# cavelandiah/BBMap

Measured on AMD Instinct MI355X. Metric: aligned_reads_per_sec, higher is better.
Workload: dtype int32

## Files before the change

bbmap_amd/csrc/pipeline.hip:

```cpp
#include <hip/hip_runtime.h>

#include <climits>

#include "bbmap_amd.h"
#include "complement.h"
#include "host_common.h"
#include "wave_prims.h"

namespace bbpipe {
using namespace wavep;

__global__ void revcomp_kernel(const bbidx_read *reads, long long n, const uint8_t *in, uint8_t *out) {
    const long long r = (long long)blockIdx.x * (blockDim.x >> 6) + (threadIdx.x >> 6);
    if (r >= n) return;
    const bbidx_read rr = reads[r];
    for (int i = threadIdx.x & 63; i < rr.len; i += 64) out[rr.bases_off + i] = (uint8_t)complement_extended(in[rr.bases_off + rr.len - 1 - i]);
}

struct RescueParams {
    const bbresc_job *jobs;
    const uint8_t *reads;
    const long long *chromOff;
    const int *chromLen, *chromMin;
    const uint8_t *refs;
    bbresc_result *results;
    long long njobs;
    int pointsMatch, pointsMatch2, useAffine, baseHitScore;
};

constexpr int RESC_WAVES = 4, RESC_MAXLEN = 608;

__global__ __launch_bounds__(64 * RESC_WAVES) void quick_rescue_kernel(const RescueParams P) {
    __shared__ __attribute__((aligned(16))) uint8_t rdbuf[RESC_WAVES][RESC_MAXLEN];
    const int wave = __builtin_amdgcn_readfirstlane(threadIdx.x >> 6), lane = threadIdx.x & 63;
    const long long jx = (long long)blockIdx.x * RESC_WAVES + wave;
    if (jx >= P.njobs) return;
    const bbresc_job jb = P.jobs[jx];
    bbresc_result res;
    res.found = 0; res.start = 0; res.stop = 0; res.score = 0; res.mismatches = 0; res.perfect = 0; res.semiperfect = 0; res.maxContig = 0;
    const int len = jb.read_len;
    if (len < 10 || len > RESC_MAXLEN - 8 || jb.chrom < 1) { if (lane == 0) { res.found = len > RESC_MAXLEN - 8 ? -2 : 0; P.results[jx] = res; } return; }
    const uint8_t *bases = P.reads + jb.read_off;
    const uint8_t *ref = P.refs + P.chromOff[jb.chrom];
    const int reflen = P.chromLen[jb.chrom], minIndex = P.chromMin[jb.chrom];
    uint8_t *rd = rdbuf[wave];
    for (int i = lane; i < len; i += 64) rd[i] = bases[i];
    wsync();
    const bool right = (jb.flags & 1) != 0;
    int lower, upper;
    if (right) { lower = max(minIndex, jb.loc); upper = min(reflen - len, jb.loc + jb.searchDist); }
    else { lower = max(minIndex, jb.loc - jb.searchDist); upper = min(reflen - len, jb.loc); }
    int minMM = jb.maxAllowedMismatches + 1, maxContig = 0, bestScore = 0, bestStart = -1, bestAbsdif = INT_MAX;
    bool finished = false;
    for (int base = 0; !finished; base += 64) {
        const int start = right ? lower + base + lane : upper - base - lane;
        const bool valid = start >= lower && start <= upper;
        if (!__ballot(valid)) break;
        const int cap = minMM;
        int mm = 0, contig = 0, cur = 0;
        const int len4 = len & ~3;
        int j = 0;
        for (; j < len4; j += 4) {
            const bool on = valid && mm <= cap;
            if (!__ballot(on)) break;
            const unsigned c4 = *(const unsigned *)(rd + j);
            if (on) {
                unsigned r4;
                __builtin_memcpy(&r4, ref + start + j, 4);
                unsigned x = c4 ^ r4;
                const unsigned isN = c4 ^ 0x4e4e4e4eu;
                const unsigned nz = (((x & 0x7f7f7f7fu) + 0x7f7f7f7fu) | x) & 0x80808080u;
                const unsigned nn = ~((((isN & 0x7f7f7f7fu) + 0x7f7f7f7fu) | isN)) & 0x80808080u;
                const unsigned bad = nz | nn;
                if (bad == 0) cur += 4;
                else {
#pragma unroll
                    for (int q = 0; q < 4; q++) {
                        if (bad & (0x80u << (8 * q))) { mm++; contig = max(contig, cur); cur = 0; } else cur++;
                    }
                }
            }
        }
        for (; j < len; j++) {
            const bool on = valid && mm <= cap;
            if (!__ballot(on)) break;
            const int c = rd[j];
            if (on) {
                const int r = ref[start + j];
                if (c != r || c == 'N') { mm++; contig = max(contig, cur); cur = 0; } else cur++;
            }
        }
        for (u64 m = __ballot(valid && mm <= cap); m; m &= m - 1) {
            const int s = __builtin_ctzll(m);
            const int st = rl(start, s), ms = rl(mm, s), ct = rl(contig, s);
            if (right ? st > upper : st < lower) { finished = true; break; }
            if (ms > minMM) continue;
            const int score = (len - ms) + ct;
            const int ad = st > jb.idealStart ? st - jb.idealStart : jb.idealStart - st;
            if (score > bestScore || (score == bestScore && ad < bestAbsdif)) {
                bestStart = st; minMM = ms; maxContig = ct; bestScore = score; bestAbsdif = ad;
                if (ms == 0) { if (right) upper = min(upper, jb.idealStart + ad); else lower = max(lower, jb.idealStart - ad); }
            }
        }
    }
    if (bestStart >= 0) {
        res.found = 1; res.start = bestStart; res.stop = bestStart + len - 1; res.mismatches = minMM; res.maxContig = maxContig;
        res.score = P.useAffine ? P.pointsMatch + P.pointsMatch2 * (len - 1 - minMM) : maxContig + P.baseHitScore * (len - minMM);
        bool perfect = true;
        int refloc = res.start, readloc = 0, N = 0;
        const int mx = min(res.stop, reflen - 1), nlimit = len / 2;
        if (res.start < 0) { N -= res.start; readloc -= res.start; refloc -= res.start; perfect = false; }
        if (res.stop >= reflen) { N += (res.stop - reflen + 1); perfect = false; }
        bool anyHard = false, anyCN = false, anyBad = false;
        if (N <= nlimit) {
            for (int j0 = 0; refloc + j0 <= mx; j0 += 64) {
                const int j = j0 + lane;
                bool bad = false, hard = false, cn = false;
                if (refloc + j <= mx) {
                    const int c = rd[readloc + j], r = ref[refloc + j];
                    bad = (c != r || c == 'N'); hard = bad && r != 'N'; cn = bad && c == 'N';
                }
                const u64 badM = __ballot(bad);
                if (badM) {
                    anyBad = true;
                    if (__ballot(hard)) { anyHard = true; break; }
                    if (__ballot(cn)) anyCN = true;
                    N += popc(badM);
                    if (N > nlimit) break;
                }
            }
            if (!anyHard && N <= nlimit) { res.semiperfect = anyCN ? 0 : 1; res.perfect = (perfect && !anyBad && !anyCN && N == 0) ? 1 : 0; }
        }
    }
    if (lane == 0) P.results[jx] = res;
}

}

extern "C" int bbpipe_revcomp_device(void *stream_, int64_t n_reads, const bbidx_read *reads, const uint8_t *bases_in, uint8_t *bases_out) {
    if (n_reads < 0) return bbfail(BBMAP_E_ARG, "bbpipe_revcomp_device: bad size");
    if (n_reads == 0) return BBMAP_OK;
    if (!reads || !bases_in || !bases_out) return bbfail(BBMAP_E_ARG, "bbpipe_revcomp_device: null buffer");
    const long long blocks = (n_reads + 3) / 4;
    hipLaunchKernelGGL(bbpipe::revcomp_kernel, dim3((unsigned)blocks), dim3(256), 0, (hipStream_t)stream_, reads, (long long)n_reads, bases_in, bases_out);
    BBHIP(hipGetLastError());
    return BBMAP_OK;
}

extern "C" int bbpipe_quick_rescue_device(void *stream_, int64_t n_jobs, const bbresc_job *jobs, const uint8_t *reads,
                                          const int64_t *chrom_off, const int32_t *chrom_len, const int32_t *chrom_min_index,
                                          const uint8_t *refs, bbresc_result *results,
                                          int32_t points_match, int32_t points_match2, int32_t use_affine, int32_t base_hit_score) {
    if (n_jobs < 0) return bbfail(BBMAP_E_ARG, "bbpipe_quick_rescue_device: bad size");
    if (n_jobs == 0) return BBMAP_OK;
    if (!jobs || !reads || !chrom_off || !chrom_len || !chrom_min_index || !refs || !results) return bbfail(BBMAP_E_ARG, "bbpipe_quick_rescue_device: null buffer");
    bbpipe::RescueParams P;
    P.jobs = jobs; P.reads = reads; P.chromOff = (const long long *)chrom_off; P.chromLen = chrom_len; P.chromMin = chrom_min_index;
    P.refs = refs; P.results = results; P.njobs = n_jobs;
    P.pointsMatch = points_match; P.pointsMatch2 = points_match2; P.useAffine = use_affine; P.baseHitScore = base_hit_score;
    const long long blocks = (n_jobs + bbpipe::RESC_WAVES - 1) / bbpipe::RESC_WAVES;
    hipLaunchKernelGGL(bbpipe::quick_rescue_kernel, dim3((unsigned)blocks), dim3(64 * bbpipe::RESC_WAVES), 0, (hipStream_t)stream_, P);
    BBHIP(hipGetLastError());
    return BBMAP_OK;
}
```

Before: 10.45 million.

## Stage reference windows in LDS for quick rescue and use branchless mismatch counting

Adds a templated staged variant of the quick-rescue kernel. Each wave cooperatively copies a 1024-start reference window into shared memory, then compares four bytes at a time using alignbyte on LDS words instead of doing unaligned global loads per lane. Per-word mismatch and contig bookkeeping becomes branchless through popcount, ffs and clz. This raises shared memory per block by about 6.5KB, which may lower occupancy, and adds restaging cost. The staged path is on by default through an environment variable.

Result: no change. 10.55 million, median of 6 (+0.9%).

```diff
diff --git a/bbmap_amd/csrc/pipeline.hip b/bbmap_amd/csrc/pipeline.hip
--- a/bbmap_amd/csrc/pipeline.hip
+++ b/bbmap_amd/csrc/pipeline.hip
@@ -29,9 +29,41 @@
 };
 
 constexpr int RESC_WAVES = 4, RESC_MAXLEN = 608;
-
-__global__ __launch_bounds__(64 * RESC_WAVES) void quick_rescue_kernel(const RescueParams P) {
+constexpr int RESC_TILE = 1024, RESC_TILE_BYTES = RESC_TILE + RESC_MAXLEN + 16, RESC_STAGE_ITERS = (RESC_TILE_BYTES / 4 + 63) / 64;
+
+__device__ inline int stage_window(uint8_t *tile, const uint8_t *ref, int reflen, int lo, int hi, int lane) {
+    const int tb = lo - (int)((uintptr_t)(ref + lo) & 3);
+    const int ndw = (hi - tb + 3) >> 2;
+    unsigned v[RESC_STAGE_ITERS];
+#pragma unroll
+    for (int i = 0; i < RESC_STAGE_ITERS; i++) {
+        const int d = i * 64 + lane, p = tb + 4 * d;
+        unsigned x = 0;
+        if (d < ndw) {
+            if (p >= 0 && p + 4 <= reflen) x = *(const unsigned *)(ref + p);
+            else {
+#pragma unroll
+                for (int q = 0; q < 4; q++) if (p + q >= 0 && p + q < reflen) x |= (unsigned)ref[p + q] << (8 * q);
+            }
+        }
+        v[i] = x;
+    }
+#pragma unroll
+    for (int i = 0; i < RESC_STAGE_ITERS; i++) {
+        const int d = i * 64 + lane;
+        if (d < ndw) ((unsigned *)tile)[d] = v[i];
+    }
+    wsync();
+    return tb;
+}
+
+template <bool STAGED> __global__ __launch_bounds__(64 * RESC_WAVES) void quick_rescue_kernel(const RescueParams P) {
     __shared__ __attribute__((aligned(16))) uint8_t rdbuf[RESC_WAVES][RESC_MAXLEN];
+    uint8_t *tile = nullptr;
+    if constexpr (STAGED) {
+        __shared__ __attribute__((aligned(16))) uint8_t tilebuf[RESC_WAVES][RESC_TILE_BYTES];
+        tile = tilebuf[__builtin_amdgcn_readfirstlane(threadIdx.x >> 6)];
+    }
     const int wave = __builtin_amdgcn_readfirstlane(threadIdx.x >> 6), lane = threadIdx.x & 63;
     const long long jx = (long long)blockIdx.x * RESC_WAVES + wave;
     if (jx >= P.njobs) return;
@@ -52,42 +84,82 @@
     else { lower = max(minIndex, jb.loc - jb.searchDist); upper = min(reflen - len, jb.loc); }
     int minMM = jb.maxAllowedMismatches + 1, maxContig = 0, bestScore = 0, bestStart = -1, bestAbsdif = INT_MAX;
     bool finished = false;
+    int tb = 0, stagedLo = 0, stagedHi = 0;
     for (int base = 0; !finished; base += 64) {
         const int start = right ? lower + base + lane : upper - base - lane;
         const bool valid = start >= lower && start <= upper;
         if (!__ballot(valid)) break;
+        if constexpr (STAGED) {
+            if ((base & (RESC_TILE - 1)) == 0) {
+                if (right) { stagedLo = lower + base; stagedHi = min(upper, stagedLo + RESC_TILE - 1) + len; }
+                else { stagedHi = upper - base + len; stagedLo = max(lower, upper - base - (RESC_TILE - 1)); }
+                tb = stage_window(tile, ref, reflen, stagedLo, stagedHi, lane);
+            }
+        }
         const int cap = minMM;
         int mm = 0, contig = 0, cur = 0;
         const int len4 = len & ~3;
         int j = 0;
-        for (; j < len4; j += 4) {
-            const bool on = valid && mm <= cap;
-            if (!__ballot(on)) break;
-            const unsigned c4 = *(const unsigned *)(rd + j);
-            if (on) {
-                unsigned r4;
-                __builtin_memcpy(&r4, ref + start + j, 4);
-                unsigned x = c4 ^ r4;
-                const unsigned isN = c4 ^ 0x4e4e4e4eu;
-                const unsigned nz = (((x & 0x7f7f7f7fu) + 0x7f7f7f7fu) | x) & 0x80808080u;
+        auto count4 = [&](unsigned c4, unsigned r4) {
+            unsigned x = c4 ^ r4;
+            const unsigned isN = c4 ^ 0x4e4e4e4eu;
+            const unsigned nz = (((x & 0x7f7f7f7fu) + 0x7f7f7f7fu) | x) & 0x80808080u;
+            const unsigned nn = ~((((isN & 0x7f7f7f7fu) + 0x7f7f7f7fu) | isN)) & 0x80808080u;
+            const unsigned bad = nz | nn;
+            if (bad == 0) cur += 4;
+            else {
+#pragma unroll
+                for (int q = 0; q < 4; q++) {
+                    if (bad & (0x80u << (8 * q))) { mm++; contig = max(contig, cur); cur = 0; } else cur++;
+                }
+            }
+        };
+        if constexpr (STAGED) {
+            const unsigned *tw = (const unsigned *)tile, *rw = (const unsigned *)rd;
+            const int o = valid ? start - tb : 0, sh = o & 3;
+            const unsigned *ta = tw + (o >> 2);
+            unsigned lo4 = ta[0];
+            for (; j < len4; j += 4) {
+                if (!__builtin_amdgcn_ballot_w64(valid && mm <= cap)) break;
+                const unsigned c4 = uni(rw[j >> 2]), hi4 = ta[(j >> 2) + 1];
+                const unsigned x = c4 ^ __builtin_amdgcn_alignbyte(hi4, lo4, sh), isN = c4 ^ 0x4e4e4e4eu;
+                lo4 = hi4;
                 const unsigned nn = ~((((isN & 0x7f7f7f7fu) + 0x7f7f7f7fu) | isN)) & 0x80808080u;
-                const unsigned bad = nz | nn;
-                if (bad == 0) cur += 4;
-                else {
-#pragma unroll
-                    for (int q = 0; q < 4; q++) {
-                        if (bad & (0x80u << (8 * q))) { mm++; contig = max(contig, cur); cur = 0; } else cur++;
-                    }
-                }
-            }
-        }
-        for (; j < len; j++) {
-            const bool on = valid && mm <= cap;
-            if (!__ballot(on)) break;
-            const int c = rd[j];
-            if (on) {
-                const int r = ref[start + j];
-                if (c != r || c == 'N') { mm++; contig = max(contig, cur); cur = 0; } else cur++;
+                const unsigned bad = ((((x & 0x7f7f7f7fu) + 0x7f7f7f7fu) | x) & 0x80808080u) | nn;
+                const int c = __builtin_popcount(bad), f = (int)min((unsigned)(__ffs((int)bad) - 1) >> 3, 4u), t = __clz((int)bad) >> 3;
+                const int head = cur + f;
+                mm += c;
+                contig = bad ? max(contig, max(head, 4 - f - t - c)) : contig;
+                cur = bad ? t : head;
+            }
+            for (; j < len; j++) {
+                const bool on = valid && mm <= cap;
+                if (!__ballot(on)) break;
+                const int c = rd[j];
+                if (on) {
+                    const int r = tile[o + j];
+                    if (c != r || c == 'N') { mm++; contig = max(contig, cur); cur = 0; } else cur++;
+                }
+            }
+        } else {
+            for (; j < len4; j += 4) {
+                const bool on = valid && mm <= cap;
+                if (!__ballot(on)) break;
+                const unsigned c4 = *(const unsigned *)(rd + j);
+                if (on) {
+                    unsigned r4;
+                    __builtin_memcpy(&r4, ref + start + j, 4);
+                    count4(c4, r4);
+                }
+            }
+            for (; j < len; j++) {
+                const bool on = valid && mm <= cap;
+                if (!__ballot(on)) break;
+                const int c = rd[j];
+                if (on) {
+                    const int r = ref[start + j];
+                    if (c != r || c == 'N') { mm++; contig = max(contig, cur); cur = 0; } else cur++;
+                }
             }
         }
         for (u64 m = __ballot(valid && mm <= cap); m; m &= m - 1) {
@@ -113,11 +185,14 @@
         if (res.stop >= reflen) { N += (res.stop - reflen + 1); perfect = false; }
         bool anyHard = false, anyCN = false, anyBad = false;
         if (N <= nlimit) {
+            if constexpr (STAGED) {
+                if (refloc < stagedLo || mx >= stagedHi) tb = stage_window(tile, ref, reflen, refloc, mx + 1, lane);
+            }
             for (int j0 = 0; refloc + j0 <= mx; j0 += 64) {
                 const int j = j0 + lane;
                 bool bad = false, hard = false, cn = false;
                 if (refloc + j <= mx) {
-                    const int c = rd[readloc + j], r = ref[refloc + j];
+                    const int c = rd[readloc + j], r = STAGED ? tile[refloc + j - tb] : ref[refloc + j];
                     bad = (c != r || c == 'N'); hard = bad && r != 'N'; cn = bad && c == 'N';
                 }
                 const u64 badM = __ballot(bad);
@@ -159,7 +234,8 @@
     P.refs = refs; P.results = results; P.njobs = n_jobs;
     P.pointsMatch = points_match; P.pointsMatch2 = points_match2; P.useAffine = use_affine; P.baseHitScore = base_hit_score;
     const long long blocks = (n_jobs + bbpipe::RESC_WAVES - 1) / bbpipe::RESC_WAVES;
-    hipLaunchKernelGGL(bbpipe::quick_rescue_kernel, dim3((unsigned)blocks), dim3(64 * bbpipe::RESC_WAVES), 0, (hipStream_t)stream_, P);
+    const auto kernel = env_int("BBPIPE_RESCUE_LDS", 1) != 0 ? bbpipe::quick_rescue_kernel<true> : bbpipe::quick_rescue_kernel<false>;
+    hipLaunchKernelGGL(kernel, dim3((unsigned)blocks), dim3(64 * bbpipe::RESC_WAVES), 0, (hipStream_t)stream_, P);
     BBHIP(hipGetLastError());
     return BBMAP_OK;
 }
```
